# leok7v/sqz

Measured on AMD Instinct MI355X. Metric: encode MB/s + decode MB/s, 32KB window, batched blocks, 1/2/4/8 MI355X, higher is better.
Workload: dtype u8; 1 GPU; 4096 x 262144 B Zipf(s=1) byte blocks, window 2^15, one independent stream per block (BASELINE.json configs[2]); total_blocks=4096, blocks_per_gpu=4096, block_bytes=262144, win_bits=15, parallelism=1 rank; the N>1 runs shard this same batch (strong scaling), finder=index, device=AMD Radeon Graphics (gfx950:sramecc+:xnack-)

## Files before the change

sqz_amd/csrc/abi.hip:

```cpp
#include "../../include/sqz/sqz.h"
#include "../../include/sqz/sqz_rc.h"
#include "sqz_kernels.h"

#include <errno.h>
#include <math.h>
#include <stdio.h>
#include <stdlib.h>
#include <string.h>

#include <atomic>
#include <mutex>
#include <vector>

namespace {

constexpr uint64_t kMaxStream = 1ull << 31;

struct DevBuf {
    void*  p = nullptr;
    size_t cap = 0;
    int reserve(size_t n) {
        if (n <= cap) { return 0; }
        if (p != nullptr) { (void)hipFree(p); p = nullptr; cap = 0; }
        size_t want = n + n / 4 + 4096;
// ... 110 lines not shown
};
Timing& timing() { static Timing t; return t; }
constexpr size_t kMaxPendingSpans = 4096;

struct SpanGuard {
    hipStream_t s; int kind; hipEvent_t a = nullptr, b = nullptr; bool on = false;
    SpanGuard(hipStream_t stream, int k) : s(stream), kind(k) {
        Timing& t = timing();
        std::lock_guard<std::mutex> g(t.mu);
        on = t.enabled;
        if (on) {
            if (hipEventCreate(&a) != hipSuccess || hipEventCreate(&b) != hipSuccess) { on = false; return; }
            (void)hipEventRecord(a, s);
        }
    }
    ~SpanGuard() {
        if (!on) { return; }
        (void)hipEventRecord(b, s);
        Timing& t = timing();
        std::lock_guard<std::mutex> g(t.mu);
        t.spans.push_back({a, b, kind});
        if (t.spans.size() >= kMaxPendingSpans) { t.drain_locked(); }
    }
};

bool writer_is_memory(const bitstream* bs) { return bs->data != NULL && bs->capacity > 0; }
bool writer_is_callback(const bitstream* bs) { return bs->data == NULL && bs->capacity == 0 && bs->output != NULL; }
bool reader_is_callback(const bitstream* bs) { return bs->data == NULL && bs->bytes == 0 && bs->input != NULL; }

void host_put_bit(bitstream* bs, int bit) {
    if (bs->error != 0) { return; }
    bs->b64 = (bs->b64 << 1) | (uint64_t)(bit & 1);
    if (++bs->bits == 64) {
        if (writer_is_memory(bs)) {
            for (int k = 0; k < 8 && bs->error == 0; k++) {
                if (bs->bytes == bs->capacity) { bs->error = E2BIG; }
                else { bs->data[bs->bytes++] = (uint8_t)(bs->b64 >> (56 - 8 * k)); }
            }
        } else if (writer_is_callback(bs)) {
            bs->error = bs->output(bs);
            if (bs->error == 0) { bs->bytes += 8; }
        } else {
            bs->error = EINVAL;
        }
        bs->bits = 0;
        bs->b64 = 0;
    }
}

void host_put_bits(bitstream* bs, uint64_t v, int n) {
    for (int b = 0; b < n && bs->error == 0; b++) { host_put_bit(bs, (int)((v >> b) & 1)); }
}

uint64_t reader_limit(const bitstream* bs) { return bs->bytes != 0 ? bs->bytes : bs->capacity; }

int host_get_bit(bitstream* bs) {
    if (bs->error != 0) { return 0; }
    if (bs->bits == 0) {
        bs->b64 = 0;
        if (bs->data != NULL) {
            const uint64_t limit = reader_limit(bs);
            for (int k = 0; k < 8 && bs->error == 0; k++) {
                if (bs->read == limit) { bs->error = E2BIG; }
                else { bs->b64 |= (uint64_t)bs->data[bs->read++] << (56 - 8 * k); }
            }
        } else if (reader_is_callback(bs)) {
            bs->error = bs->input(bs);
            if (bs->error == 0) { bs->read += 8; }
        } else {
            bs->error = EINVAL;
        }
        bs->bits = 64;
    }
    const int bit = (int)(bs->b64 >> 63);
    bs->b64 <<= 1;
    bs->bits--;
    return bit;
}

uint64_t host_get_bits(bitstream* bs, int n) {
    uint64_t v = 0;
    for (int b = 0; b < n && bs->error == 0; b++) { v |= (uint64_t)host_get_bit(bs) << b; }
    return v;
}

uint64_t load_be64(const uint8_t* p) {
    uint64_t w = 0;
    for (int k = 0; k < 8; k++) { w = (w << 8) | p[k]; }
    return w;
}

void store_be64(uint8_t* p, uint64_t w) {
    for (int k = 0; k < 8; k++) { p[k] = (uint8_t)(w >> (56 - 8 * k)); }
}

bool window_ok(uint32_t w) { return w >= 2 && w <= 32768; }

int scan_waves() {
    static const int w = [] {
        const char* e = getenv("SQZ_SCAN_WAVES");
        const int v = e != NULL ? atoi(e) : 4;
        return (v == 1 || v == 2 || v == 4 || v == 8) ? v : 4;
    }();
    return w;
}

int check_offsets(const uint64_t* off, uint32_t n, bool need8) {
    for (uint32_t b = 0; b < n; b++) {
        if (off[b + 1] < off[b] || off[b + 1] - off[b] > kMaxStream) { return EINVAL; }
        if (need8 && (off[b] & 7u) != 0) { return EINVAL; }
    }
    return 0;
}

uint64_t align_up(uint64_t v, uint64_t a) { return (v + a - 1) / a * a; }

std::atomic<int> g_finder{-1};
int finder_default() {
    int f = g_finder.load(std::memory_order_relaxed);
    if (f < 0) {
        const char* e = getenv("SQZ_FINDER");
        const int chosen = (e != NULL && strcmp(e, "scan") == 0) ? 0 : 1;
        f = g_finder.compare_exchange_strong(f, chosen) ? chosen : g_finder.load();
    }
    return f;
}

int decode_waves_for(uint32_t n_blocks) {
    static const int forced = [] { const char* e = getenv("SQZ_DECODE_WAVES"); return e != NULL ? atoi(e) : 0; }();
    if (forced == 1 || forced == 2 || forced == 4 || forced == 8) { return forced; }
    int cus = ctx().cus;
    if (cus <= 0) { cus = 256; }
    if ((uint64_t)n_blocks <= (uint64_t)cus * 2) { return 8; }
    return (uint64_t)n_blocks <= (uint64_t)cus * 4 ? 4 : 1;
}

uint32_t match_groups_for(uint64_t avg_block_bytes) {
    static const int div = [] { const char* e = getenv("SQZ_MATCH_DIV"); const int v = e != NULL ? atoi(e) : 1024; return v >= 256 ? v : 1024; }();
    uint64_t g = (avg_block_bytes + div - 1) / div;
    if (g < 1) { g = 1; }
    if (g > 65535) { g = 65535; }
    return (uint32_t)g;
}

void run_stage1(int finder, const uint8_t* d_in, const uint64_t* d_in_off, uint32_t n,
                uint32_t window, uint32_t* tokens, uint32_t* counts,
                uint32_t* work_a, uint32_t* work_m, uint64_t avg_block, uint64_t slots,
                hipStream_t st) {
    if (finder == 0 || work_a == nullptr || work_m == nullptr) {
        SpanGuard g(st, SQZ_HIP_K_LZ77_SCAN);
        sqzk::launch_lz77_scan(d_in, d_in_off, n, window, tokens, counts, scan_waves(), slots, st);
    } else {
        { SpanGuard g(st, SQZ_HIP_K_INDEX_SORT);
          sqzk::launch_index_sort(d_in, d_in_off, n, work_a, work_m , nullptr, slots, st); }
        { SpanGuard g(st, SQZ_HIP_K_INDEX_MATCH);
          sqzk::launch_index_match(d_in, d_in_off, n, window, work_a, work_m,
                                   match_groups_for(avg_block), slots, st); }
        { SpanGuard g(st, SQZ_HIP_K_INDEX_PARSE);
          sqzk::launch_index_parse(d_in, d_in_off, n, work_m, tokens, counts, slots, st); }
    }
}

void run_encode(int finder, const uint8_t* d_in, const uint64_t* d_in_off, uint32_t n,
                uint32_t window, uint32_t* tokens, uint32_t* counts, uint32_t* work_a,
                uint32_t* work_m, uint64_t avg_block, uint8_t* d_out, const uint64_t* d_out_off,
                uint64_t* d_out_bytes, int32_t* d_err, uint64_t prefix_acc, int prefix_fill,
                uint64_t slots, sqz_block_stats* d_stats, hipStream_t st) {
    run_stage1(finder, d_in, d_in_off, n, window, tokens, counts, work_a, work_m, avg_block, slots, st);
    SpanGuard g(st, SQZ_HIP_K_HUFFMAN_EMIT);
    sqzk::launch_huffman_emit(tokens, d_in_off, counts, d_out, d_out_off, d_out_bytes, d_err, n,
                              prefix_acc, prefix_fill, d_stats, st);
}

int encode_host(Lane& c, hipStream_t st, const uint8_t* in, const uint64_t* in_off, uint32_t n,
                       uint32_t window, uint8_t* out, const uint64_t* out_off,
                       uint64_t* out_bytes, int32_t* err,
                       uint64_t prefix_acc, int prefix_fill, uint64_t* tokens_total) {
    const uint64_t in_base = in_off[0], out_base = out_off[0];
    const uint64_t total_in = in_off[n] - in_base, total_out = out_off[n] - out_base;
    std::vector<uint64_t> io(n + 1), oo(n + 1);
    for (uint32_t b = 0; b <= n; b++) { io[b] = in_off[b] - in_base; oo[b] = out_off[b] - out_base; }

    int e;
    if ((e = c.in.reserve(total_in + 16)) || (e = c.out.reserve(total_out + 16)) ||
        (e = c.in_off.reserve((n + 1) * 8)) || (e = c.out_off.reserve((n + 1) * 8)) ||
        (e = c.tok_count.reserve((size_t)n * 4)) ||
        (e = c.work_a.reserve((total_in + 64) * 4)) || (e = c.work_m.reserve((total_in + 64) * 4)) ||
        (e = c.out_bytes.reserve((size_t)n * 8)) || (e = c.err.reserve((size_t)n * 4))) {
        return e;
    }
    if (total_in > 0) { HIP_TRY(hipMemcpyAsync(c.in.p, in + in_base, total_in, hipMemcpyHostToDevice, st)); }
    HIP_TRY(hipMemcpyAsync(c.in_off.p, io.data(), (n + 1) * 8, hipMemcpyHostToDevice, st));
    HIP_TRY(hipMemcpyAsync(c.out_off.p, oo.data(), (n + 1) * 8, hipMemcpyHostToDevice, st));
    uint64_t widest = 0;
    for (uint32_t b = 0; b < n; b++) { widest = io[b + 1] - io[b] > widest ? io[b + 1] - io[b] : widest; }
    run_encode(finder_default(), (const uint8_t*)c.in.p, (const uint64_t*)c.in_off.p, n, window,
               (uint32_t*)c.work_a.p , (uint32_t*)c.tok_count.p,
               (uint32_t*)c.work_a.p, (uint32_t*)c.work_m.p, widest, (uint8_t*)c.out.p, (const uint64_t*)c.out_off.p,
               (uint64_t*)c.out_bytes.p, (int32_t*)c.err.p, prefix_acc, prefix_fill, total_in + 64, nullptr, st);
    HIP_TRY(hipGetLastError());
    HIP_TRY(hipMemcpyAsync(out_bytes, c.out_bytes.p, (size_t)n * 8, hipMemcpyDeviceToHost, st));
    HIP_TRY(hipMemcpyAsync(err, c.err.p, (size_t)n * 4, hipMemcpyDeviceToHost, st));
    HIP_TRY(hipStreamSynchronize(st));
    std::vector<uint64_t> dense_off(n + 1);
    dense_off[0] = 0;
    for (uint32_t b = 0; b < n; b++) { dense_off[b + 1] = dense_off[b] + ((out_bytes[b] + 7) & ~7ull); }
    const uint64_t dense_total = dense_off[n];
    if (dense_total > 0) {
        if (n == 1) {
            HIP_TRY(hipMemcpyAsync(out + out_off[0], c.out.p, out_bytes[0], hipMemcpyDeviceToHost, st));
        } else {
            if ((e = c.dense.reserve(dense_total + 16)) || (e = c.dense_off.reserve((n + 1) * 8))) { return e; }
            HIP_TRY(hipMemcpyAsync(c.dense_off.p, dense_off.data(), (n + 1) * 8, hipMemcpyHostToDevice, st));
            sqzk::launch_compact_blocks((const uint8_t*)c.out.p, (const uint64_t*)c.out_off.p,
                                        (const uint64_t*)c.out_bytes.p, n, (uint8_t*)c.dense.p,
                                        (const uint64_t*)c.dense_off.p, dense_total / n, st);
            HIP_TRY(hipGetLastError());
            if (c.host_dense.size() < dense_total) { c.host_dense.resize(dense_total); }
            HIP_TRY(hipMemcpyAsync(c.host_dense.data(), c.dense.p, dense_total, hipMemcpyDeviceToHost, st));
            HIP_TRY(hipStreamSynchronize(st));
            for (uint32_t b = 0; b < n; b++) {
                memcpy(out + out_off[b], c.host_dense.data() + dense_off[b], out_bytes[b]);
            }
        }
    }
    if (tokens_total != nullptr) {
        std::vector<uint32_t> tc(n);
        HIP_TRY(hipMemcpyAsync(tc.data(), c.tok_count.p, (size_t)n * 4, hipMemcpyDeviceToHost, st));
        HIP_TRY(hipStreamSynchronize(st));
        uint64_t sum = 0;
        for (uint32_t b = 0; b < n; b++) { sum += tc[b]; }
        *tokens_total = sum;
    }
    HIP_TRY(hipStreamSynchronize(st));
    return 0;
}

int decode_host(Lane& c, hipStream_t st, const uint8_t* in, const uint64_t* in_off, uint32_t n,
                uint8_t* out, const uint64_t* out_off, int32_t* err,
                uint64_t start_bit, uint64_t* end_bit) {
    const uint64_t in_base = in_off[0], out_base = out_off[0];
    const uint64_t total_in = in_off[n] - in_base, total_out = out_off[n] - out_base;
    std::vector<uint64_t> io(n + 1), oo(n + 1);
    for (uint32_t b = 0; b <= n; b++) { io[b] = in_off[b] - in_base; oo[b] = out_off[b] - out_base; }
    int e;
    if ((e = c.in.reserve(total_in + 16)) || (e = c.out.reserve(total_out + 16)) ||
        (e = c.in_off.reserve((n + 1) * 8)) || (e = c.out_off.reserve((n + 1) * 8)) ||
        (e = c.err.reserve((size_t)n * 4)) || (e = c.end_bit.reserve((size_t)n * 8)) ||
        (e = c.tokens.reserve((total_out + 64) * 4)) || (e = c.tok_count.reserve((size_t)n * 4))) {
        return e;
    }
    if (total_in > 0) { HIP_TRY(hipMemcpyAsync(c.in.p, in + in_base, total_in, hipMemcpyHostToDevice, st)); }
    HIP_TRY(hipMemcpyAsync(c.in_off.p, io.data(), (n + 1) * 8, hipMemcpyHostToDevice, st));
    HIP_TRY(hipMemcpyAsync(c.out_off.p, oo.data(), (n + 1) * 8, hipMemcpyHostToDevice, st));
    {
        SpanGuard g(st, SQZ_HIP_K_ENTROPY_DECODE);
        sqzk::launch_entropy_decode((const uint8_t*)c.in.p, (const uint64_t*)c.in_off.p,
                                    (const uint64_t*)c.out_off.p, (uint32_t*)c.tokens.p,
                                    (uint32_t*)c.tok_count.p, (int32_t*)c.err.p,
                                    (uint64_t*)c.end_bit.p, n, start_bit, decode_waves_for(n), st);
    }
    {
        SpanGuard g(st, SQZ_HIP_K_LZ_EXPAND);
        sqzk::launch_lz_expand((const uint32_t*)c.tokens.p, (const uint32_t*)c.tok_count.p,
                               (uint8_t*)c.out.p, (const uint64_t*)c.out_off.p, n, st);
    }
    HIP_TRY(hipGetLastError());
    HIP_TRY(hipMemcpyAsync(err, c.err.p, (size_t)n * 4, hipMemcpyDeviceToHost, st));
    if (total_out > 0) {
        HIP_TRY(hipMemcpyAsync(out + out_base, c.out.p, total_out, hipMemcpyDeviceToHost, st));
    }
    if (end_bit != nullptr) {
        HIP_TRY(hipMemcpyAsync(end_bit, c.end_bit.p, (size_t)n * 8, hipMemcpyDeviceToHost, st));
    }
    HIP_TRY(hipStreamSynchronize(st));
    return 0;
}

}

extern "C" {

const char* sqz_version(void) { return "sqz_amd 0.1 (gfx950; H0 semantics, H1 names)"; }

int sqz_hip_device_info(char* name, size_t name_cap, int* compute_units,
                        uint64_t* lds_bytes_per_cu) {
    Ctx& c = ctx();
    std::lock_guard<std::mutex> g(c.mu);
    const int e = probe_locked(c);
    if (e != 0) { return e; }
    if (name != NULL && name_cap > 0) { snprintf(name, name_cap, "%s", c.name); }
    if (compute_units != NULL) { *compute_units = c.cus; }
    if (lds_bytes_per_cu != NULL) { *lds_bytes_per_cu = c.lds; }
    return 0;
}

uint64_t sqz_bound(uint64_t bytes) { return (2 * bytes + 1024 + 7) & ~(uint64_t)7; }

int sqz_file_words(const uint8_t* in, uint64_t bytes, uint8_t* out) {
    if ((bytes & 7u) != 0 || (bytes != 0 && (in == NULL || out == NULL))) { return EINVAL; }
    for (uint64_t k = 0; k < bytes; k += 8) {
        uint64_t w = 0;
        for (int j = 0; j < 8; j++) { w = (w << 8) | in[k + j]; }
        memcpy(out + k, &w, 8);
    }
    return 0;
}
// ... 512 lines not shown
```

sqz_amd/csrc/lz77_index.hip:

```cpp
#include "sqz_device.h"
#include "sqz_kernels.h"

namespace sqzk {

constexpr int kSharedGiveUp = 8;
constexpr int kXcds = 8;
constexpr int kSortThreads = 1024;
constexpr int kSortWaves = kSortThreads / kWave;

constexpr int kSortTile = 4 * kSortThreads;

constexpr int kSortBins = 1024;
struct SortLds {
    uint32_t elem[kSortTile];
    uint16_t dig[kSortTile];
    uint16_t cnt[kSortWaves][kSortBins];
    uint32_t gbase[3][kSortBins];
    uint32_t tstart[kSortBins];
    uint32_t total[kSortBins];
};

struct __attribute__((packed)) U32u { uint32_t v; };

__device__ __forceinline__ uint32_t load_u32_unaligned(const uint8_t* p) {
    return reinterpret_cast<const U32u*>(p)->v;
}

__device__ __forceinline__ uint64_t peers_of(uint32_t digit, bool valid, int bits) {
    uint64_t peers = __ballot(valid);
#pragma unroll
    for (int bit = 0; bit < 10; bit++) {
        if (bit < bits) {
            const bool set = (digit >> bit) & 1u;
            const uint64_t m = __ballot(set);
            peers &= set ? m : ~m;
        }
    }
    return peers;
}

__device__ __forceinline__ uint32_t lanes_below(uint64_t mask) {
    return __builtin_amdgcn_mbcnt_hi((uint32_t)(mask >> 32),
                                     __builtin_amdgcn_mbcnt_lo((uint32_t)mask, 0u));
}

__global__ __launch_bounds__(kSortThreads)
void index_sort_kernel(const uint8_t* __restrict__ in,
                       const uint64_t* __restrict__ in_off,
                       uint32_t n_blocks,
                       uint32_t* __restrict__ buf_a,
                       uint32_t* __restrict__ buf_b,
                       uint32_t* __restrict__ tmp,
                       uint64_t slots) {
    __shared__ SortLds lds;
    const uint32_t b = blockIdx.x;
    if (b >= n_blocks || in_off[b + 1] > slots) { return; }
    const int tid = threadIdx.x;
    const int lane = tid & (kWave - 1);
    const int wave = __builtin_amdgcn_readfirstlane(tid >> 6);

    const uint8_t* src = in + in_off[b];
    const uint64_t bytes = in_off[b + 1] - in_off[b];
    if (bytes < 3) { return; }
    const uint32_t count = (uint32_t)(bytes - 2);
    uint32_t* const pa = buf_a + in_off[b];
    uint32_t* const pb = buf_b + in_off[b];
    (void)tmp;
    auto key_of = [&](uint32_t k) {
        return (uint64_t)k + 4 <= bytes ? (__builtin_bswap32(load_u32_unaligned(src + k)) >> 8)
                                        : (((uint32_t)src[k] << 16) | ((uint32_t)src[k + 1] << 8) | (uint32_t)src[k + 2]);
    };
    const bool small = bytes <= (1u << 18);
    const bool carry = bytes <= (1u << 24);
    const int w0 = small ? 10 : 8, w1 = small ? 7 : 8, w2 = small ? 7 : 8;
    const int s1 = w0, s2 = w0 + w1;
    const uint32_t m0 = (1u << w0) - 1u, m1 = (1u << w1) - 1u;
    for (int d = tid; d < 3 * kSortBins; d += kSortThreads) { (&lds.gbase[0][0])[d] = 0; }
    __syncthreads();
    for (uint32_t k = (uint32_t)tid; k < count; k += (uint32_t)kSortThreads) {
        const uint32_t key = key_of(k);
        atomicAdd(&lds.gbase[0][key & m0], 1u);
        atomicAdd(&lds.gbase[1][(key >> s1) & m1], 1u);
        atomicAdd(&lds.gbase[2][key >> s2], 1u);
    }
    __syncthreads();
    if (wave < 3) {
        uint32_t* const g = lds.gbase[wave];
        const int per = (1 << (wave == 0 ? w0 : wave == 1 ? w1 : w2)) / kWave;
        uint32_t sum = 0;
        for (int j = 0; j < per; j++) { sum += g[per * lane + j]; }
        uint32_t excl = wave_scan(sum) - sum;
        for (int j = 0; j < per; j++) { const uint32_t v = g[per * lane + j]; g[per * lane + j] = excl; excl += v; }
    }
    __syncthreads();

    for (int pass = 0; pass < 3; pass++) {
        const uint32_t* from = pass == 1 ? pa : pb;
        uint32_t* to = pass == 1 ? pb : pa;
        uint32_t* const gbase = lds.gbase[pass];
        const int bits = pass == 0 ? w0 : pass == 1 ? w1 : w2;
        const int bins = 1 << bits;

        auto load_rows = [&](uint32_t tile, uint32_t (&elem)[4], uint32_t (&digit)[4], bool (&valid)[4]) {
            uint32_t pos[4];
#pragma unroll
            for (int j = 0; j < 4; j++) {
                const uint32_t k = tile + (uint32_t)(wave * 256 + j * kWave + lane);
                valid[j] = k < count;
                pos[j] = valid[j] ? (pass == 0 ? k : from[k]) : 0u;
            }
#pragma unroll
            for (int j = 0; j < 4; j++) {
                digit[j] = 0; elem[j] = pos[j];
                if (!valid[j]) { continue; }
                if (small) {
                    if (pass == 0) {
                        const uint32_t key = key_of(pos[j]);
                        digit[j] = key & m0;
                        elem[j] = pos[j] | ((key >> 10) << 18);
                    } else if (pass == 1) {
                        digit[j] = (pos[j] >> 18) & m1;
                    } else {
                        digit[j] = pos[j] >> 25;
                        elem[j] = pos[j] & 0x3FFFFu;
                    }
                } else if (pass == 0) {
                    digit[j] = src[pos[j] + 2];
                } else if (pass == 1) {
                    const uint32_t w = (uint32_t)src[pos[j]] | ((uint32_t)src[pos[j] + 1] << 8);
                    digit[j] = w >> 8;
                    if (carry) { elem[j] = pos[j] | ((w & 0xFFu) << 24); }
                } else {
                    digit[j] = carry ? (pos[j] >> 24) : (uint32_t)src[pos[j]];
                    if (carry) { elem[j] = pos[j] & 0x00FFFFFFu; }
                }
            }
        };

        for (uint32_t tile = 0; tile < count; tile += (uint32_t)kSortTile) {
            const uint32_t n_tile = count - tile < (uint32_t)kSortTile ? count - tile : (uint32_t)kSortTile;
            for (int d = lane; d < bins; d += kWave) { lds.cnt[wave][d] = 0; }
            uint32_t elem[4], digit[4], wrank[4];
            bool valid[4];
            load_rows(tile, elem, digit, valid);
#pragma unroll
            for (int j = 0; j < 4; j++) {
                const uint64_t peers = peers_of(digit[j], valid[j], bits);
                const uint32_t rank = lanes_below(peers);
                wrank[j] = valid[j] ? (uint32_t)lds.cnt[wave][digit[j]] + rank : 0u;
                __builtin_amdgcn_wave_barrier();
                if (valid[j] && rank == 0) {
                    lds.cnt[wave][digit[j]] = (uint16_t)(lds.cnt[wave][digit[j]] + (uint32_t)__builtin_popcountll(peers));
                }
                __builtin_amdgcn_wave_barrier();
            }
            __syncthreads();
            uint32_t tcount = 0;
            if (tid < bins) {
                for (int w = 0; w < kSortWaves; w++) {
                    const uint32_t c = lds.cnt[w][tid];
                    lds.cnt[w][tid] = (uint16_t)tcount;
                    tcount += c;
                }
                lds.total[tid] = tcount;
            }
            __syncthreads();
            if (wave == 0) {
                const int per = bins / kWave;
                uint32_t sum = 0;
                for (int j = 0; j < per; j++) { sum += lds.total[per * lane + j]; }
                uint32_t excl = wave_scan(sum) - sum;
                for (int j = 0; j < per; j++) { lds.tstart[per * lane + j] = excl; excl += lds.total[per * lane + j]; }
            }
            __syncthreads();
#pragma unroll
            for (int j = 0; j < 4; j++) {
                if (valid[j]) {
                    const uint32_t slot = lds.tstart[digit[j]] + (uint32_t)lds.cnt[wave][digit[j]] + wrank[j];
                    if (slot < (uint32_t)kSortTile) {
                        lds.elem[slot] = elem[j];
                        lds.dig[slot] = (uint16_t)digit[j];
                    }
                }
            }
            __syncthreads();
#pragma unroll
            for (int j = 0; j < 4; j++) {
                const uint32_t slot = (uint32_t)(j * kSortThreads + tid);
                if (slot < n_tile) {
                    const uint32_t d = lds.dig[slot];
                    const uint32_t dest = gbase[d] + (slot - lds.tstart[d]);
                    if (dest < count) { to[dest] = lds.elem[slot]; }
                }
            }
            __syncthreads();
            if (tid < bins) { gbase[tid] += tcount; }
        }
        __threadfence_block();
        __syncthreads();
    }
}

__global__ __launch_bounds__(256)
void index_match_kernel(const uint8_t* __restrict__ in,
                        const uint64_t* __restrict__ in_off,
                        uint32_t n_blocks, uint32_t window,
                        const uint32_t* __restrict__ sorted,
                        uint32_t* __restrict__ match, uint32_t groups, uint64_t slots) {
    const uint32_t xcd = blockIdx.x % (uint32_t)kXcds;
    const uint32_t local = blockIdx.x / (uint32_t)kXcds;
    const uint32_t b = (local / groups) * (uint32_t)kXcds + xcd;
    const uint32_t group = local % groups;
    if (b >= n_blocks || in_off[b + 1] > slots) { return; }
    const uint8_t* src = in + in_off[b];
    const uint64_t bytes = in_off[b + 1] - in_off[b];
    if (bytes < 3) { return; }
    const uint32_t n = (uint32_t)bytes;
    const uint32_t count = n - 2;
    const uint32_t* S = sorted + in_off[b];
    uint32_t* M = match + in_off[b];

    const int lane = (int)(threadIdx.x & (kWave - 1));
    const uint32_t pages = (count + (uint32_t)kWave - 1u) / (uint32_t)kWave;
    const uint32_t waves = groups * (blockDim.x / (uint32_t)kWave);
    const uint32_t per_wave = (pages + waves - 1u) / waves;
    const uint32_t wave_id = group * (blockDim.x / (uint32_t)kWave) + (threadIdx.x - (uint32_t)lane) / (uint32_t)kWave;
    const uint32_t page_lo = wave_id * per_wave;
    const uint32_t page_hi = page_lo + per_wave < pages ? page_lo + per_wave : pages;
    auto load16 = [&](uint32_t at, uint32_t& w0, uint32_t& w1, uint32_t& w2, uint32_t& w3) {
        if (at + 16 <= n) {
            w0 = load_u32_unaligned(src + at); w1 = load_u32_unaligned(src + at + 4);
            w2 = load_u32_unaligned(src + at + 8); w3 = load_u32_unaligned(src + at + 12);
        } else {
            uint32_t w[4] = {0, 0, 0, 0};
            for (uint32_t k = 0; k < 16 && at + k < n; k++) { w[k >> 2] |= (uint32_t)src[at + k] << (8 * (k & 3)); }
            w0 = w[0]; w1 = w[1]; w2 = w[2]; w3 = w[3];
        }
    };
    uint32_t prev_i = 0, prev0 = 0, prev1 = 0, prev2 = 0, prev3 = 0;
    if (page_lo > 0 && page_lo < page_hi) {
        prev_i = S[(page_lo - 1u) * (uint32_t)kWave + (uint32_t)lane];
        load16(prev_i, prev0, prev1, prev2, prev3);
    }
    for (uint32_t pg = page_lo; pg < page_hi; pg++) {
        const uint32_t r0 = pg * (uint32_t)kWave;
        const bool have_prev = pg > 0;
        const uint32_t r = r0 + (uint32_t)lane;
        const bool valid = r < count;
        const uint32_t i = valid ? S[r] : 0u;
        const uint32_t cap = (n - i) < (uint32_t)kLenMax ? (n - i) : (uint32_t)kLenMax;
        const uint32_t reach = i < window - 1 ? i : window - 1;
        uint32_t own0 = 0, own1 = 0, own2 = 0, own3 = 0;
        if (valid) { load16(i, own0, own1, own2, own3); }
        const uint32_t key = own0 & 0x00FFFFFFu;
        uint32_t best = 0, dist = 0;
        auto walk = [&](uint32_t q_from) {
            if (q_from == 0 || best >= cap) { return; }
            auto inside = [&](uint32_t r) {
                const uint32_t p = S[r];
                if (p + 4 > n) { return false; }
                return (load_u32_unaligned(src + p) & 0x00FFFFFFu) == key && i - p <= reach;
            };
            uint32_t q_lo;
            {
                uint32_t d = 4, bad = 0, good = q_from;
                bool open = true;
                while (open) {
                    if (d >= q_from) { bad = 0; open = false; if (inside(0)) { good = 0; } else { bad = 1; } }
                    else if (inside(q_from - d)) { good = q_from - d; d <<= 1; }
                    else { bad = q_from - d + 1; open = false; }
                }
                uint32_t lo = bad, hi = good;
                while (lo < hi) {
                    const uint32_t mid = lo + ((hi - lo) >> 1);
                    if (inside(mid)) { hi = mid; } else { lo = mid + 1; }
                }
                q_lo = lo;
            }
            uint8_t own_next = best >= (uint32_t)kLenMin ? src[i + best] : (uint8_t)0;
            for (uint32_t q = q_from; q > q_lo && best < cap; ) {
                q--;
                const uint32_t p = S[q];
                if (best >= (uint32_t)kLenMin && src[p + best] != own_next) { continue; }
                uint32_t k = 3;
                while (k < cap) {
                    if (i + k + 4 <= n) {
                        const uint32_t x = load_u32_unaligned(src + p + k) ^ load_u32_unaligned(src + i + k);
                        if (x != 0) { k += (uint32_t)__builtin_ctz(x) >> 3; break; }
                        k += 4;
                    } else {
                        if (src[p + k] != src[i + k]) { break; }
                        k++;
                    }
                }
                if (k > cap) { k = cap; }
                if (k > best) {
                    best = k; dist = i - p;
                    if (best < cap) { own_next = src[i + best]; }
                }
            }
        };
        const uint32_t key0 = (uint32_t)__builtin_amdgcn_readfirstlane((int)key);
        if (__ballot(valid && key == key0 && i + 16 <= n) == ~0ull) {
            bool done = false, deferred = false;
            uint32_t resume = 0;
            uint32_t page_base = r0, page = i, pb0 = own0, pb1 = own1, pb2 = own2, pb3 = own3;
            for (int64_t c = (int64_t)r0 + kWave - 2; c >= 0; c--) {
                if (c < (int64_t)page_base) {
                    page_base -= (uint32_t)kWave;
                    page = S[page_base + (uint32_t)lane];
                    load16(page, pb0, pb1, pb2, pb3);
                }
                const int at = (int)(c - (int64_t)page_base);
                const uint32_t pc = (uint32_t)__builtin_amdgcn_readlane((int)page, at);
                const bool below = (int64_t)r > c;
                const uint32_t d = i - pc;
                if (below && d > reach) { done = true; }
                if (__ballot(!done) == 0) { break; }
                const uint32_t c0 = (uint32_t)__builtin_amdgcn_readlane((int)pb0, at);
                if ((c0 & 0x00FFFFFFu) != key0) { break; }
                const uint32_t c1 = (uint32_t)__builtin_amdgcn_readlane((int)pb1, at);
                const uint32_t c2 = (uint32_t)__builtin_amdgcn_readlane((int)pb2, at);
                const uint32_t c3 = (uint32_t)__builtin_amdgcn_readlane((int)pb3, at);
                const uint32_t x0 = own0 ^ c0, x1 = own1 ^ c1, x2 = own2 ^ c2, x3 = own3 ^ c3;
                uint32_t len = x0 != 0 ? ((uint32_t)__builtin_ctz(x0) >> 3)
                             : x1 != 0 ? 4u + ((uint32_t)__builtin_ctz(x1) >> 3)
                             : x2 != 0 ? 8u + ((uint32_t)__builtin_ctz(x2) >> 3)
                             : x3 != 0 ? 12u + ((uint32_t)__builtin_ctz(x3) >> 3) : 16u;
                const bool want = below && !done;
                if (want && len == 16u && cap > 16u) {
                    deferred = true;
                    resume = (uint32_t)c + 1u;
                    done = true;
                } else {
                    if (len > cap) { len = cap; }
                    if (want && len > best) {
                        best = len; dist = d;
                        if (best >= cap) { done = true; }
                    }
                }
                if (__builtin_popcountll(__ballot(deferred)) >= kSharedGiveUp) {
                    if (!done) {
                        deferred = true;
                        resume = below ? (uint32_t)c : r;
                        done = true;
                    }
                    break;
                }
            }
            if (deferred) { walk(resume); }
            M[i] = best >= (uint32_t)kLenMin ? ((best << 16) | dist) : (key & 0xFFu);
            prev_i = i; prev0 = own0; prev1 = own1; prev2 = own2; prev3 = own3;
            continue;
// ... 12 lines not shown
            uint32_t c1 = (uint32_t)__builtin_amdgcn_ds_bpermute(addr, (int)own1);
            const bool back = __ballot(!done && !in_cur) != 0;
            if (back) {
                const uint32_t qc = (uint32_t)__builtin_amdgcn_ds_bpermute(addr, (int)prev_i);
                const uint32_t q0 = (uint32_t)__builtin_amdgcn_ds_bpermute(addr, (int)prev0);
                const uint32_t q1 = (uint32_t)__builtin_amdgcn_ds_bpermute(addr, (int)prev1);
                pc = in_cur ? pc : qc; c0 = in_cur ? c0 : q0; c1 = in_cur ? c1 : q1;
            }
            const uint32_t x0 = own0 ^ c0, x1 = own1 ^ c1;
            if (!done && (x0 & 0x00FFFFFFu) != 0) { done = true; }
            const uint32_t d = i - pc;
            if (!done && d > reach) { done = true; }
            uint32_t len = x0 != 0 ? ((uint32_t)__builtin_ctz(x0) >> 3) : x1 != 0 ? 4u + ((uint32_t)__builtin_ctz(x1) >> 3) : 8u;
            if (__ballot(!done && len == 8u && cap > 8u) != 0) {
                uint32_t c2 = (uint32_t)__builtin_amdgcn_ds_bpermute(addr, (int)own2);
                uint32_t c3 = (uint32_t)__builtin_amdgcn_ds_bpermute(addr, (int)own3);
                if (back) {
                    const uint32_t q2 = (uint32_t)__builtin_amdgcn_ds_bpermute(addr, (int)prev2);
                    const uint32_t q3 = (uint32_t)__builtin_amdgcn_ds_bpermute(addr, (int)prev3);
                    c2 = in_cur ? c2 : q2; c3 = in_cur ? c3 : q3;
                }
                const uint32_t x2 = own2 ^ c2, x3 = own3 ^ c3;
                if (len == 8u) {
                    len = x2 != 0 ? 8u + ((uint32_t)__builtin_ctz(x2) >> 3) : x3 != 0 ? 12u + ((uint32_t)__builtin_ctz(x3) >> 3) : 16u;
                }
            }
            if (!done) {
                if (len == 16u && cap > 16u) {
                    later = true;
                    resume = r - (uint32_t)k + 1u;
                    done = true;
                } else {
                    if (len > cap) { len = cap; }
                    if (len > best) {
                        best = len; dist = d;
                        if (best >= cap) { done = true; }
                    }
                    if (!done && k == kWave) {
                        later = true;
                        resume = r - (uint32_t)kWave;
                        done = true;
                    }
                }
            }
        }
        if (later) { walk(resume); }
        if (valid) { M[i] = best >= (uint32_t)kLenMin ? ((best << 16) | dist) : (key & 0xFFu); }
        prev_i = i; prev0 = own0; prev1 = own1; prev2 = own2; prev3 = own3;
    }
}

constexpr int kChunk = 32;
constexpr int kTile = kChunk * kWave;
constexpr int kChunkRow = kChunk + 1;

struct ParseLds {
    uint32_t m[kChunkRow * kWave];
};

__device__ __forceinline__ uint32_t parse_slot(uint32_t k) { return k + (k / (uint32_t)kChunk); }

__device__ __forceinline__ uint32_t parse_step(uint32_t w) {
    const uint32_t len = w >> 16;
    return len != 0 ? len : 1u;
}

__global__ __launch_bounds__(kWave)
void index_parse_kernel(const uint8_t* __restrict__ in,
                        const uint64_t* __restrict__ in_off,
                        uint32_t n_blocks,
                        const uint32_t* __restrict__ match,
                        uint32_t* __restrict__ tokens,
                        uint32_t* __restrict__ tok_count, uint64_t slots) {
    __shared__ ParseLds lds;
    const uint32_t b = blockIdx.x;
    if (b >= n_blocks) { return; }
    const int lane = threadIdx.x;
    if (in_off[b + 1] > slots) {
        if (lane == 0) { tok_count[b] = kRefused; }
        return;
    }
    const uint8_t* src = in + in_off[b];
    const uint64_t bytes = in_off[b + 1] - in_off[b];
    const uint32_t* M = match + in_off[b];
    uint32_t* tok = tokens + in_off[b];

    uint32_t ntok = 0;
    uint32_t entry = 0;
    for (uint64_t tile = 0; tile < bytes; tile += (uint64_t)kTile) {
        const uint64_t left = bytes - tile;
        const uint32_t have = left < (uint64_t)kTile ? (uint32_t)left : (uint32_t)kTile;
        if (entry >= have) { entry -= (uint32_t)kTile; continue; }
        __syncthreads();
        for (uint32_t k = lane; k < have; k += kWave) {
            lds.m[parse_slot(k)] = (tile + k + 2 < bytes) ? M[tile + k] : (uint32_t)src[tile + k];
        }
        __syncthreads();

        const uint32_t lo = (uint32_t)lane * (uint32_t)kChunk;
        const uint32_t room = have > lo ? (have - lo < (uint32_t)kChunk ? have - lo : (uint32_t)kChunk) : 0u;
        const uint32_t* row = &lds.m[lane * kChunkRow];
        uint32_t guess = 0;
        uint32_t p = 0;
        while (p < room) {
            guess |= 1u << p;
            const uint32_t w = row[p];
            p += parse_step(w);
        }
        const uint32_t guess_out = lo + p;

        uint32_t mine = 0;
        uint32_t e = entry;
        for (int l = 0; l < kWave; l++) {
            const uint32_t clo = (uint32_t)l * (uint32_t)kChunk;
            if (clo >= have) { break; }
            const uint32_t chi = clo + (uint32_t)kChunk < have ? clo + (uint32_t)kChunk : have;
            if (e >= chi) { continue; }
            const uint32_t g = (uint32_t)__builtin_amdgcn_readlane((int)guess, l);
            const uint32_t gout = (uint32_t)__builtin_amdgcn_readlane((int)guess_out, l);
            uint32_t real = 0;
            uint32_t q = e - clo;
            const uint32_t croom = chi - clo;
            for (;;) {
                if ((g >> q) & 1u) {
                    real |= g & ~((1u << q) - 1u);
                    e = gout;
                    break;
                }
                real |= 1u << q;
                const uint32_t w = (uint32_t)__builtin_amdgcn_readfirstlane((int)lds.m[l * kChunkRow + (int)q]);
                q += parse_step(w);
                if (q >= croom) { e = clo + q; break; }
            }
            if (lane == l) { mine = real; }
        }
        entry = e - (uint32_t)kTile;

        const uint32_t cnt = (uint32_t)__builtin_popcount(mine);
        const uint32_t incl = wave_scan(cnt);
        uint32_t at = ntok + incl - cnt;
        uint32_t bits = mine;
        while (bits != 0) {
            const uint32_t k = (uint32_t)__builtin_ctz(bits);
            bits &= bits - 1u;
            const uint32_t w = row[k];
            tok[at++] = (w >> 16) != 0 ? (kTokMatch | w) : (w & 0xFFu);
        }
        ntok += (uint32_t)__builtin_amdgcn_readlane((int)incl, kWave - 1);
    }
    if (lane == 0) { tok_count[b] = ntok; }
}

void launch_index_sort(const uint8_t* in, const uint64_t* in_off, uint32_t n_blocks,
                       uint32_t* buf_a, uint32_t* buf_b, uint32_t* tmp, uint64_t slots,
                       hipStream_t stream) {
    if (n_blocks == 0) { return; }
    hipLaunchKernelGGL(index_sort_kernel, dim3(n_blocks), dim3(kSortThreads), 0, stream,
                       in, in_off, n_blocks, buf_a, buf_b, tmp, slots);
}

void launch_index_match(const uint8_t* in, const uint64_t* in_off, uint32_t n_blocks,
                        uint32_t window, const uint32_t* sorted, uint32_t* match,
                        uint32_t match_groups, uint64_t slots, hipStream_t stream) {
    if (n_blocks == 0) { return; }
    if (match_groups < 1) { match_groups = 1; }
    const uint32_t rounded = (n_blocks + (uint32_t)kXcds - 1) / (uint32_t)kXcds * (uint32_t)kXcds;
    while ((uint64_t)match_groups * rounded > 0x7FFFFFFFull) { match_groups = (match_groups + 1) / 2; }
    hipLaunchKernelGGL(index_match_kernel, dim3(rounded * match_groups), dim3(256), 0, stream,
                       in, in_off, n_blocks, window, sorted, match, match_groups, slots);
}

void launch_index_parse(const uint8_t* in, const uint64_t* in_off, uint32_t n_blocks,
                        const uint32_t* match, uint32_t* tokens, uint32_t* tok_count,
                        uint64_t slots, hipStream_t stream) {
    if (n_blocks == 0) { return; }
    hipLaunchKernelGGL(index_parse_kernel, dim3(n_blocks), dim3(kWave), 0, stream,
                       in, in_off, n_blocks, match, tokens, tok_count, slots);
}

}
```

sqz_amd/csrc/sqz_kernels.h:

```cpp
#pragma once

#include <hip/hip_runtime.h>
#include <stdint.h>

#include "../../include/sqz/sqz.h"

namespace sqzk {

void launch_lz77_scan(const uint8_t* in, const uint64_t* in_off, uint32_t n_blocks,
                      uint32_t window, uint32_t* tokens, uint32_t* tok_count,
                      int waves_per_stream, uint64_t slots, hipStream_t stream);

void launch_index_sort(const uint8_t* in, const uint64_t* in_off, uint32_t n_blocks,
                       uint32_t* buf_a, uint32_t* buf_b, uint32_t* tmp, uint64_t slots,
                       hipStream_t stream);
void launch_index_match(const uint8_t* in, const uint64_t* in_off, uint32_t n_blocks,
                        uint32_t window, const uint32_t* sorted, uint32_t* match,
                        uint32_t match_groups, uint64_t slots, hipStream_t stream);
void launch_index_parse(const uint8_t* in, const uint64_t* in_off, uint32_t n_blocks,
                        const uint32_t* match, uint32_t* tokens, uint32_t* tok_count,
                        uint64_t slots, hipStream_t stream);

void launch_huffman_emit(const uint32_t* tokens, const uint64_t* tok_off,
                         const uint32_t* tok_count, uint8_t* out,
                         const uint64_t* out_off, uint64_t* out_bytes,
                         int32_t* err, uint32_t n_blocks,
                         uint64_t prefix_acc, int prefix_fill, sqz_block_stats* stats,
                         hipStream_t stream);

void launch_tree_debug(const int32_t* symbols, uint32_t count, int which, int batch, uint32_t* dump,
                       hipStream_t stream);

void launch_entropy_decode(const uint8_t* in, const uint64_t* in_off, const uint64_t* out_off,
                           uint32_t* tokens, uint32_t* tok_count, int32_t* err, uint64_t* end_bit,
                           uint32_t n_blocks, uint64_t start_bit, int waves, hipStream_t stream);
void launch_lz_expand(const uint32_t* tokens, const uint32_t* tok_count, uint8_t* out,
                      const uint64_t* out_off, uint32_t n_blocks, hipStream_t stream);

void launch_rc_encode(const uint8_t* in, const uint64_t* in_off, uint8_t* out, const uint64_t* out_off,
                      uint64_t* out_bytes, int32_t* err, uint32_t n_blocks, hipStream_t stream);
void launch_rc_decode(const uint8_t* in, const uint64_t* in_off, uint8_t* out, const uint64_t* out_off,
                      uint64_t* out_bytes, uint64_t* consumed, int32_t* err, uint32_t n_blocks, int dry_error,
                      hipStream_t stream);

void launch_compact_blocks(const uint8_t* src, const uint64_t* src_off, const uint64_t* bytes,
                           uint32_t n_blocks, uint8_t* dst, const uint64_t* dst_off,
                           uint64_t avg_bytes, hipStream_t stream);

}
```

Baseline: 13680 MB/s.

## Restructure index radix sort passes with prefetch, parallel digit scan, fewer barriers

Moves each radix-sort pass into a templated function specialised on digit width. The pass prefetches the next tile's loads while the current tile is ranked, and replaces the serial per-bin loop over waves with a parallel scan across all threads. Placement now uses a single per-digit delta table. Other changes: the ballot-based peer mask works on 32-bit halves, the count rows are padded, and the histogram reads eight bytes per thread. Adds optional cycle-counter instrumentation under SQZ_STATS, at the cost of more complex code and clamped out-of-range loads.

```diff
diff --git a/sqz_amd/csrc/abi.hip b/sqz_amd/csrc/abi.hip
--- a/sqz_amd/csrc/abi.hip
+++ b/sqz_amd/csrc/abi.hip
@@ -286,7 +286,7 @@
         sqzk::launch_lz77_scan(d_in, d_in_off, n, window, tokens, counts, scan_waves(), slots, st);
     } else {
         { SpanGuard g(st, SQZ_HIP_K_INDEX_SORT);
-          sqzk::launch_index_sort(d_in, d_in_off, n, work_a, work_m , nullptr, slots, st); }
+          sqzk::launch_index_sort(d_in, d_in_off, n, work_a, work_m , slots, st); }
         { SpanGuard g(st, SQZ_HIP_K_INDEX_MATCH);
           sqzk::launch_index_match(d_in, d_in_off, n, window, work_a, work_m,
                                    match_groups_for(avg_block), slots, st); }
diff --git a/sqz_amd/csrc/lz77_index.hip b/sqz_amd/csrc/lz77_index.hip
--- a/sqz_amd/csrc/lz77_index.hip
+++ b/sqz_amd/csrc/lz77_index.hip
@@ -11,13 +11,14 @@
 constexpr int kSortTile = 4 * kSortThreads;
 
 constexpr int kSortBins = 1024;
+constexpr int kSortCntRow = kSortBins + 2;
 struct SortLds {
     uint32_t elem[kSortTile];
     uint16_t dig[kSortTile];
-    uint16_t cnt[kSortWaves][kSortBins];
+    uint16_t cnt[kSortWaves][kSortCntRow];
     uint32_t gbase[3][kSortBins];
-    uint32_t tstart[kSortBins];
-    uint32_t total[kSortBins];
+    uint32_t delta[kSortBins];
+    uint32_t wtot[kSortWaves];
 };
 
 struct __attribute__((packed)) U32u { uint32_t v; };
@@ -27,21 +28,179 @@
 }
 
 __device__ __forceinline__ uint64_t peers_of(uint32_t digit, bool valid, int bits) {
-    uint64_t peers = __ballot(valid);
+    const uint64_t all = __ballot(valid);
+    uint32_t lo = (uint32_t)all, hi = (uint32_t)(all >> 32);
 #pragma unroll
     for (int bit = 0; bit < 10; bit++) {
         if (bit < bits) {
-            const bool set = (digit >> bit) & 1u;
-            const uint64_t m = __ballot(set);
-            peers &= set ? m : ~m;
-        }
-    }
-    return peers;
+            const uint32_t mine = (uint32_t)((int32_t)(digit << (31 - bit)) >> 31);
+            const uint64_t m = __ballot(mine != 0u);
+            lo &= ~((uint32_t)m ^ mine);
+            hi &= ~((uint32_t)(m >> 32) ^ mine);
+        }
+    }
+    return ((uint64_t)hi << 32) | lo;
 }
 
 __device__ __forceinline__ uint32_t lanes_below(uint64_t mask) {
     return __builtin_amdgcn_mbcnt_hi((uint32_t)(mask >> 32),
                                      __builtin_amdgcn_mbcnt_lo((uint32_t)mask, 0u));
+}
+
+__device__ __forceinline__ uint32_t sort_key(const uint8_t* src, uint64_t bytes, uint32_t k) {
+    return (uint64_t)k + 4 <= bytes ? (__builtin_bswap32(load_u32_unaligned(src + k)) >> 8)
+                                    : (((uint32_t)src[k] << 16) | ((uint32_t)src[k + 1] << 8) | (uint32_t)src[k + 2]);
+}
+
+typedef uint32_t __attribute__((may_alias)) SortCntPair;
+
+struct SortSec {
+#ifdef SQZ_STATS
+    uint64_t t[8] = {0, 0, 0, 0, 0, 0, 0, 0};
+    uint64_t last = 0;
+#endif
+};
+#ifdef SQZ_STATS
+#define SORT_SEC(s, k) { const uint64_t n_ = __builtin_readcyclecounter(); (s).t[k] += n_ - (s).last; (s).last = n_; }
+#define SORT_SEC_LOADS(s, k) { asm volatile("s_waitcnt vmcnt(0)" ::: "memory"); SORT_SEC(s, k) }
+#else
+#define SORT_SEC(s, k)
+#define SORT_SEC_LOADS(s, k)
+#endif
+
+template <int kBits, bool kSmall>
+__device__ __forceinline__ void sort_pass(SortLds& lds, const int pass, const uint8_t* __restrict__ src,
+                                          const uint64_t bytes, const uint32_t count, const bool carry,
+                                          const uint32_t* __restrict__ from, uint32_t* __restrict__ to, SortSec& sec) {
+    constexpr int kDigits = 1 << kBits;
+    constexpr int kTpd = kSortThreads / kDigits;
+    constexpr int kWpt = kSortWaves / kTpd;
+    const int tid = threadIdx.x;
+    const int lane = tid & (kWave - 1);
+    const int wave = __builtin_amdgcn_readfirstlane(tid >> 6);
+    const bool first = kSmall ? kBits == 10 : pass == 0;
+    uint32_t* const gbase = lds.gbase[pass];
+
+    auto fetch = [&](uint32_t tile, uint32_t (&raw)[4]) {
+#pragma unroll
+        for (int j = 0; j < 4; j++) {
+            const uint32_t k = tile + (uint32_t)(wave * 256 + j * kWave + lane);
+            if (first) {
+                const uint32_t last = (uint32_t)(bytes - 4);
+                raw[j] = load_u32_unaligned(src + (k < last ? k : last));
+            } else {
+                raw[j] = from[k < count ? k : count - 1u];
+            }
+        }
+    };
+    auto key_from = [&](uint32_t raw, uint32_t k) {
+        const uint32_t be = __builtin_bswap32(raw);
+        return (uint64_t)k + 4 <= bytes ? be >> 8 : be & 0x00FFFFFFu;
+    };
+    auto decode = [&](uint32_t tile, const uint32_t (&raw)[4], uint32_t (&elem)[4], uint32_t (&digit)[4], bool (&valid)[4]) {
+#pragma unroll
+        for (int j = 0; j < 4; j++) {
+            const uint32_t k = tile + (uint32_t)(wave * 256 + j * kWave + lane);
+            valid[j] = k < count;
+            const uint32_t pos = valid[j] ? (first ? k : raw[j]) : 0u;
+            digit[j] = 0; elem[j] = pos;
+            if (!valid[j]) { continue; }
+            if (kSmall) {
+                if (first) {
+                    const uint32_t key = key_from(raw[j], k);
+                    digit[j] = key & 0x3FFu;
+                    elem[j] = pos | ((key >> 10) << 18);
+                } else if (pass == 1) {
+                    digit[j] = (pos >> 18) & 0x7Fu;
+                } else {
+                    digit[j] = pos >> 25;
+                    elem[j] = pos & 0x3FFFFu;
+                }
+            } else if (first) {
+                digit[j] = key_from(raw[j], k) & 0xFFu;
+            } else if (pass == 1) {
+                const uint32_t w = (uint32_t)src[pos] | ((uint32_t)src[pos + 1] << 8);
+                digit[j] = w >> 8;
+                if (carry) { elem[j] = pos | ((w & 0xFFu) << 24); }
+            } else {
+                digit[j] = carry ? (pos >> 24) : (uint32_t)src[pos];
+                if (carry) { elem[j] = pos & 0x00FFFFFFu; }
+            }
+        }
+    };
+
+    uint32_t ahead[4], elem[4], digit[4], wrank[4];
+    bool valid[4];
+    fetch(0u, ahead);
+    decode(0u, ahead, elem, digit, valid);
+    SORT_SEC_LOADS(sec, 1)
+    for (uint32_t tile = 0; tile < count; tile += (uint32_t)kSortTile) {
+        const uint32_t n_tile = count - tile < (uint32_t)kSortTile ? count - tile : (uint32_t)kSortTile;
+        fetch(tile + (uint32_t)kSortTile, ahead);
+        {
+            SortCntPair* const row = reinterpret_cast<SortCntPair*>(lds.cnt[wave]);
+            for (int d = lane; d < kDigits / 2; d += kWave) { row[d] = 0u; }
+        }
+#pragma unroll
+        for (int j = 0; j < 4; j++) {
+            const uint64_t peers = peers_of(digit[j], valid[j], kBits);
+            const uint32_t rank = lanes_below(peers);
+            wrank[j] = valid[j] ? (uint32_t)lds.cnt[wave][digit[j]] + rank : 0u;
+            __builtin_amdgcn_wave_barrier();
+            if (valid[j] && rank == 0) {
+                lds.cnt[wave][digit[j]] = (uint16_t)(lds.cnt[wave][digit[j]] + (uint32_t)__builtin_popcountll(peers));
+            }
+            __builtin_amdgcn_wave_barrier();
+        }
+        lds_barrier();
+        SORT_SEC(sec, 2)
+        const int sd = tid / kTpd;
+        const int sw = (tid % kTpd) * kWpt;
+        uint32_t c[kWpt], sum = 0;
+#pragma unroll
+        for (int i = 0; i < kWpt; i++) { c[i] = lds.cnt[sw + i][sd]; sum += c[i]; }
+        const uint32_t incl = wave_scan(sum);
+        if (lane == kWave - 1) { lds.wtot[wave] = incl; }
+        lds_barrier();
+        SORT_SEC(sec, 3)
+        uint32_t at = wave_scan(lane < wave ? lds.wtot[lane] : 0u);
+        at = (uint32_t)__builtin_amdgcn_readlane((int)at, kWave - 1) + incl - sum;
+        const uint32_t run = at;
+#pragma unroll
+        for (int i = 0; i < kWpt; i++) { lds.cnt[sw + i][sd] = (uint16_t)at; at += c[i]; }
+        const uint32_t run_end = kTpd > 1 ? (uint32_t)__shfl((int)at, lane | (kTpd - 1)) : at;
+        if (tid % kTpd == 0) {
+            const uint32_t g = gbase[sd];
+            lds.delta[sd] = g - run;
+            gbase[sd] = g + (run_end - run);
+        }
+        lds_barrier();
+        SORT_SEC(sec, 4)
+#pragma unroll
+        for (int j = 0; j < 4; j++) {
+            if (valid[j]) {
+                const uint32_t slot = (uint32_t)lds.cnt[wave][digit[j]] + wrank[j];
+                if (slot < (uint32_t)kSortTile) {
+                    lds.elem[slot] = elem[j];
+                    lds.dig[slot] = (uint16_t)digit[j];
+                }
+            }
+        }
+        lds_barrier();
+        SORT_SEC(sec, 5)
+#pragma unroll
+        for (int j = 0; j < 4; j++) {
+            const uint32_t slot = (uint32_t)(j * kSortThreads + tid);
+            const uint32_t s = slot < n_tile ? slot : n_tile - 1u;
+            const uint32_t dest = s + lds.delta[lds.dig[s]];
+            to[dest < count ? dest : count - 1u] = lds.elem[s];
+        }
+        SORT_SEC(sec, 6)
+        decode(tile + (uint32_t)kSortTile, ahead, elem, digit, valid);
+        SORT_SEC_LOADS(sec, 1)
+    }
+    __threadfence_block();
+    __syncthreads();
 }
 
 __global__ __launch_bounds__(kSortThreads)
@@ -50,7 +209,6 @@
                        uint32_t n_blocks,
                        uint32_t* __restrict__ buf_a,
                        uint32_t* __restrict__ buf_b,
-                       uint32_t* __restrict__ tmp,
                        uint64_t slots) {
     __shared__ SortLds lds;
     const uint32_t b = blockIdx.x;
@@ -65,24 +223,39 @@
     const uint32_t count = (uint32_t)(bytes - 2);
     uint32_t* const pa = buf_a + in_off[b];
     uint32_t* const pb = buf_b + in_off[b];
-    (void)tmp;
-    auto key_of = [&](uint32_t k) {
-        return (uint64_t)k + 4 <= bytes ? (__builtin_bswap32(load_u32_unaligned(src + k)) >> 8)
-                                        : (((uint32_t)src[k] << 16) | ((uint32_t)src[k + 1] << 8) | (uint32_t)src[k + 2]);
-    };
+    if (bytes == 3) {
+        if (tid == 0) { pa[0] = 0u; }
+        return;
+    }
     const bool small = bytes <= (1u << 18);
     const bool carry = bytes <= (1u << 24);
     const int w0 = small ? 10 : 8, w1 = small ? 7 : 8, w2 = small ? 7 : 8;
     const int s1 = w0, s2 = w0 + w1;
     const uint32_t m0 = (1u << w0) - 1u, m1 = (1u << w1) - 1u;
+    SortSec sec;
+#ifdef SQZ_STATS
+    sec.last = __builtin_readcyclecounter();
+    const uint64_t sec_begin = sec.last;
+#endif
     for (int d = tid; d < 3 * kSortBins; d += kSortThreads) { (&lds.gbase[0][0])[d] = 0; }
     __syncthreads();
-    for (uint32_t k = (uint32_t)tid; k < count; k += (uint32_t)kSortThreads) {
-        const uint32_t key = key_of(k);
+    auto count_key = [&](uint32_t key) {
         atomicAdd(&lds.gbase[0][key & m0], 1u);
         atomicAdd(&lds.gbase[1][(key >> s1) & m1], 1u);
         atomicAdd(&lds.gbase[2][key >> s2], 1u);
-    }
+    };
+    const uint32_t quads = bytes >= 8 ? (uint32_t)((bytes - 8) / 4) + 1u : 0u;
+    if ((uint32_t)tid < quads) {
+        uint32_t lo = load_u32_unaligned(src + 4u * (uint32_t)tid), hi = load_u32_unaligned(src + 4u * (uint32_t)tid + 4u);
+        for (uint32_t q = (uint32_t)tid; q < quads; q += (uint32_t)kSortThreads) {
+            const uint64_t eight = ((uint64_t)hi << 32) | lo;
+            const uint32_t nq = q + (uint32_t)kSortThreads < quads ? q + (uint32_t)kSortThreads : q;
+            lo = load_u32_unaligned(src + 4u * nq); hi = load_u32_unaligned(src + 4u * nq + 4u);
+#pragma unroll
+            for (int j = 0; j < 4; j++) { count_key(__builtin_bswap32((uint32_t)(eight >> (8 * j))) >> 8); }
+        }
+    }
+    for (uint32_t k = 4u * quads + (uint32_t)tid; k < count; k += (uint32_t)kSortThreads) { count_key(sort_key(src, bytes, k)); }
     __syncthreads();
     if (wave < 3) {
         uint32_t* const g = lds.gbase[wave];
@@ -93,112 +266,26 @@
         for (int j = 0; j < per; j++) { const uint32_t v = g[per * lane + j]; g[per * lane + j] = excl; excl += v; }
     }
     __syncthreads();
-
-    for (int pass = 0; pass < 3; pass++) {
-        const uint32_t* from = pass == 1 ? pa : pb;
-        uint32_t* to = pass == 1 ? pb : pa;
-        uint32_t* const gbase = lds.gbase[pass];
-        const int bits = pass == 0 ? w0 : pass == 1 ? w1 : w2;
-        const int bins = 1 << bits;
-
-        auto load_rows = [&](uint32_t tile, uint32_t (&elem)[4], uint32_t (&digit)[4], bool (&valid)[4]) {
-            uint32_t pos[4];
-#pragma unroll
-            for (int j = 0; j < 4; j++) {
-                const uint32_t k = tile + (uint32_t)(wave * 256 + j * kWave + lane);
-                valid[j] = k < count;
-                pos[j] = valid[j] ? (pass == 0 ? k : from[k]) : 0u;
-            }
-#pragma unroll
-            for (int j = 0; j < 4; j++) {
-                digit[j] = 0; elem[j] = pos[j];
-                if (!valid[j]) { continue; }
-                if (small) {
-                    if (pass == 0) {
-                        const uint32_t key = key_of(pos[j]);
-                        digit[j] = key & m0;
-                        elem[j] = pos[j] | ((key >> 10) << 18);
-                    } else if (pass == 1) {
-                        digit[j] = (pos[j] >> 18) & m1;
-                    } else {
-                        digit[j] = pos[j] >> 25;
-                        elem[j] = pos[j] & 0x3FFFFu;
-                    }
-                } else if (pass == 0) {
-                    digit[j] = src[pos[j] + 2];
-                } else if (pass == 1) {
-                    const uint32_t w = (uint32_t)src[pos[j]] | ((uint32_t)src[pos[j] + 1] << 8);
-                    digit[j] = w >> 8;
-                    if (carry) { elem[j] = pos[j] | ((w & 0xFFu) << 24); }
-                } else {
-                    digit[j] = carry ? (pos[j] >> 24) : (uint32_t)src[pos[j]];
-                    if (carry) { elem[j] = pos[j] & 0x00FFFFFFu; }
-                }
-            }
-        };
-
-        for (uint32_t tile = 0; tile < count; tile += (uint32_t)kSortTile) {
-            const uint32_t n_tile = count - tile < (uint32_t)kSortTile ? count - tile : (uint32_t)kSortTile;
-            for (int d = lane; d < bins; d += kWave) { lds.cnt[wave][d] = 0; }
-            uint32_t elem[4], digit[4], wrank[4];
-            bool valid[4];
-            load_rows(tile, elem, digit, valid);
-#pragma unroll
-            for (int j = 0; j < 4; j++) {
-                const uint64_t peers = peers_of(digit[j], valid[j], bits);
-                const uint32_t rank = lanes_below(peers);
-                wrank[j] = valid[j] ? (uint32_t)lds.cnt[wave][digit[j]] + rank : 0u;
-                __builtin_amdgcn_wave_barrier();
-                if (valid[j] && rank == 0) {
-                    lds.cnt[wave][digit[j]] = (uint16_t)(lds.cnt[wave][digit[j]] + (uint32_t)__builtin_popcountll(peers));
-                }
-                __builtin_amdgcn_wave_barrier();
-            }
-            __syncthreads();
-            uint32_t tcount = 0;
-            if (tid < bins) {
-                for (int w = 0; w < kSortWaves; w++) {
-                    const uint32_t c = lds.cnt[w][tid];
-                    lds.cnt[w][tid] = (uint16_t)tcount;
-                    tcount += c;
-                }
-                lds.total[tid] = tcount;
-            }
-            __syncthreads();
-            if (wave == 0) {
-                const int per = bins / kWave;
-                uint32_t sum = 0;
-                for (int j = 0; j < per; j++) { sum += lds.total[per * lane + j]; }
-                uint32_t excl = wave_scan(sum) - sum;
-                for (int j = 0; j < per; j++) { lds.tstart[per * lane + j] = excl; excl += lds.total[per * lane + j]; }
-            }
-            __syncthreads();
-#pragma unroll
-            for (int j = 0; j < 4; j++) {
-                if (valid[j]) {
-                    const uint32_t slot = lds.tstart[digit[j]] + (uint32_t)lds.cnt[wave][digit[j]] + wrank[j];
-                    if (slot < (uint32_t)kSortTile) {
-                        lds.elem[slot] = elem[j];
-                        lds.dig[slot] = (uint16_t)digit[j];
-                    }
-                }
-            }
-            __syncthreads();
-#pragma unroll
-            for (int j = 0; j < 4; j++) {
-                const uint32_t slot = (uint32_t)(j * kSortThreads + tid);
-                if (slot < n_tile) {
-                    const uint32_t d = lds.dig[slot];
-                    const uint32_t dest = gbase[d] + (slot - lds.tstart[d]);
-                    if (dest < count) { to[dest] = lds.elem[slot]; }
-                }
-            }
-            __syncthreads();
-            if (tid < bins) { gbase[tid] += tcount; }
-        }
-        __threadfence_block();
-        __syncthreads();
-    }
+    SORT_SEC(sec, 0)
+
+    if (small) {
+        sort_pass<10, true>(lds, 0, src, bytes, count, carry, pb, pa, sec);
+        for (int pass = 1; pass < 3; pass++) {
+            sort_pass<7, true>(lds, pass, src, bytes, count, carry, pass == 1 ? pa : pb, pass == 1 ? pb : pa, sec);
+        }
+    } else {
+        for (int pass = 0; pass < 3; pass++) {
+            sort_pass<8, false>(lds, pass, src, bytes, count, carry, pass == 1 ? pa : pb, pass == 1 ? pb : pa, sec);
+        }
+    }
+#ifdef SQZ_STATS
+    if (tid == 0 && b == 1) {
+        printf("sort block 1: cycles %llu: hist %llu; tiles: loads %llu rank %llu scan_a %llu scan_b %llu place %llu copy_out %llu\n",
+               (unsigned long long)(sec.last - sec_begin), (unsigned long long)sec.t[0], (unsigned long long)sec.t[1],
+               (unsigned long long)sec.t[2], (unsigned long long)sec.t[3], (unsigned long long)sec.t[4],
+               (unsigned long long)sec.t[5], (unsigned long long)sec.t[6]);
+    }
+#endif
 }
 
 __global__ __launch_bounds__(256)
@@ -517,11 +604,11 @@
 }
 
 void launch_index_sort(const uint8_t* in, const uint64_t* in_off, uint32_t n_blocks,
-                       uint32_t* buf_a, uint32_t* buf_b, uint32_t* tmp, uint64_t slots,
+                       uint32_t* buf_a, uint32_t* buf_b, uint64_t slots,
                        hipStream_t stream) {
     if (n_blocks == 0) { return; }
     hipLaunchKernelGGL(index_sort_kernel, dim3(n_blocks), dim3(kSortThreads), 0, stream,
-                       in, in_off, n_blocks, buf_a, buf_b, tmp, slots);
+                       in, in_off, n_blocks, buf_a, buf_b, slots);
 }
 
 void launch_index_match(const uint8_t* in, const uint64_t* in_off, uint32_t n_blocks,
diff --git a/sqz_amd/csrc/sqz_kernels.h b/sqz_amd/csrc/sqz_kernels.h
--- a/sqz_amd/csrc/sqz_kernels.h
+++ b/sqz_amd/csrc/sqz_kernels.h
@@ -12,7 +12,7 @@
                       int waves_per_stream, uint64_t slots, hipStream_t stream);
 
 void launch_index_sort(const uint8_t* in, const uint64_t* in_off, uint32_t n_blocks,
-                       uint32_t* buf_a, uint32_t* buf_b, uint32_t* tmp, uint64_t slots,
+                       uint32_t* buf_a, uint32_t* buf_b, uint64_t slots,
                        hipStream_t stream);
 void launch_index_match(const uint8_t* in, const uint64_t* in_off, uint32_t n_blocks,
                         uint32_t window, const uint32_t* sorted, uint32_t* match,
```

Result: faster. 14370 MB/s, median of 6 (+5.1%).
